# SYNCC-IN/hyperscanning-signal-analysis

Hardware: AMD Instinct MI355X
Metric: MVAR+ffDTF windows/sec, 2x32-ch dyad p=8, 256 freqs (higher is better)
Workload: dtype f64; 1 GPU; C2: 1 dyad(s)/GPU, 2x32 ch @500 Hz, 10 min, 2 s windows 50% overlap (599 windows per dyad), MVAR p=8, 256 freqs 0.5-128 Hz; dyads_per_gpu=1, k1=hop blocks summed once, shared by the overlapping windows (hop 500), k2=block Levinson-Whittle recursion, one workgroup per window, one launch, normalisation=inside K3 (rows of window w by workgroups of window w+lag), parallelism=dyad-sharded x1, gather=none

## Files before the change

### hyperscanning_signal_analysis_amd/csrc/capi.hip

```cpp
#include "../../include/hypermvar.h"
#include "hmv_kernels.h"

#include <atomic>
#include <cmath>
#include <cstdio>
#include <cstdlib>
#include <cstring>

namespace {
thread_local char g_err[256] = "";

int fail(int code, const char* msg) {
  snprintf(g_err, sizeof(g_err), "%s", msg);
  return code;
}
int pad_of(int m) { return (m < 1 || m > HMV_MAX_CHANNELS) ? -1 : ((m + 15) / 16) * 16; }
inline hipStream_t S(void* s) { return reinterpret_cast<hipStream_t>(s); }
inline size_t align256(size_t b) { return (b + 255) & ~size_t(255); }

constexpr int N_TUNE = 6;
struct TuneRange { long long lo, hi; };
constexpr TuneRange kTuneRange[N_TUNE] = {{0, 0}, {0, 1 << 20}, {0, 3}, {0, 2}, {0, 4}, {0, 140000}};
long long env_knob(const char* name, int key) {
  const char* e = getenv(name);
// ... 741 lines not shown
      hmv::LagcovEnsArgs ea{};
      ea.x = a.x; ea.rec_stride = a.rec_stride; ea.ld = a.ld; ea.T = a.ens->T;
      ea.trial_rec = reinterpret_cast<const long long*>(a.ens->trial_rec);
      ea.trial_start = reinterpret_cast<const long long*>(a.ens->trial_start);
      ea.group_ptr = reinterpret_cast<const long long*>(a.ens->group_ptr);
      ea.item_group = reinterpret_cast<const long long*>(a.item_rec + i0);
      ea.item_offset = reinterpret_cast<const long long*>(a.item_start + i0);
      ea.n_items = c; ea.m = a.m; ea.n = a.n; ea.p = a.p; ea.R = R;
      if (ens_shared) {
        ea.it0 = i0; ea.nwin = a.grid_nwin; ea.hop = a.grid_hop; ea.k = (int)(a.n / a.grid_hop); ea.Q = Qb;
      }
      if (a.ens->split) {
        ea.trial_rec_b = reinterpret_cast<const long long*>(a.ens->trial_rec_b);
        ea.trial_start_b = reinterpret_cast<const long long*>(a.ens->trial_start_b);
        ea.split = a.ens->split; ea.R_base = a.ens->R_base;
        ea.item_base = a.ens->item_base ? reinterpret_cast<const long long*>(a.ens->item_base + i0) : nullptr;
        rc = hmv::launch_lagcov_ensemble_split(ea, mp, st0);
      } else {
        rc = hmv::launch_lagcov_ensemble(ea, mp, ens_shared, st0);
      }
    } else if (a.pairs) {
      hmv::LagcovPairsArgs pa{};
      pa.x = a.x; pa.rec_stride = a.rec_stride; pa.ld = a.ld;
      pa.rec_a = reinterpret_cast<const long long*>(a.item_rec + i0);
      pa.rec_b = reinterpret_cast<const long long*>(a.pairs->rec_b + i0);
      pa.item_start = reinterpret_cast<const long long*>(a.item_start + i0);
      pa.n_items = c; pa.m = a.m; pa.n = a.n; pa.p = a.p; pa.split = a.pairs->split; pa.R = R;
      pa.R_base = a.pairs->R_base;
      pa.base_a = a.pairs->R_base ? reinterpret_cast<const long long*>(a.pairs->base_a + i0) : nullptr;
      pa.base_b = a.pairs->R_base ? reinterpret_cast<const long long*>(a.pairs->base_b + i0) : nullptr;
      rc = hmv::launch_lagcov_pairs(pa, mp, st0);
    } else if (a.mix) {
      hmv::LagcovMixArgs ma{};
      ma.Rt = a.mix->Rt; ma.W = a.mix->W; ma.scale = a.mix->scale; ma.n_trials = a.mix->n_trials; ma.n_win = a.mix->n_win;
      ma.it0 = i0; ma.n_items = c; ma.m = a.m; ma.m_pad = mp; ma.p = a.p; ma.R = R;
      rc = hmv::launch_lagcov_mix(ma, st0);
    } else if (regular) {
      for (int64_t it = i0; it < i0 + c && rc == 0;) {
        const int64_t rec = it / a.grid_nwin, w0 = it - rec * a.grid_nwin;
        const int64_t run = ((a.grid_nwin - w0) < (i0 + c - it)) ? (a.grid_nwin - w0) : (i0 + c - it);
        rc = hmv_lagcov_regular_f64(a.x + rec * a.rec_stride, a.ld, a.grid_T, a.grid_first + w0 * a.grid_hop, a.grid_hop,
                                    run, a.m, a.n, a.p, R + (size_t)(it - i0) * (a.p + 1) * t, Qb, st0);
        it += run;
      }
    } else {
      rc = hmv_lagcov_f64(a.x, a.rec_stride, a.ld, a.item_rec + i0, a.item_start + i0, c, a.m, a.n, a.p, R, st0);
    }
    if (rc) break;
    if (automatic) {
      hmv::YwArgs ya{};
      ya.R = R; ya.n_items = c; ya.m = a.m; ya.p = a.p; ya.ws = ws; ya.ar = ar_c; ya.V = V_c; ya.info = a.info_yw + i0;
      ya.tiled = -1;
      hmv::YwAutoArgs sel{};
      sel.n = a.n; sel.crit_c = crit_factor(a.crit, a.n); sel.order_out = a.order_out + i0;
      sel.crit_out = a.crit_out ? a.crit_out + (size_t)i0 * a.p : nullptr;
      rc = hmv::launch_yw_auto(ya, sel, mp, st0);
      if (rc) break;
    }
    const bool ldl = (a.flags & (HMV_FLAG_YW_TILED | HMV_FLAG_YW_ONE_LAUNCH)) || hmv::tuning(HMV_TUNE_YW_FORM) == 1;
    const bool tiled = (a.flags & HMV_FLAG_YW_TILED) || (ldl && !(a.flags & HMV_FLAG_YW_ONE_LAUNCH) && mp == 64 && c >= 128);
    const int64_t yw_flags = (a.flags & ~(int64_t)(HMV_FLAG_YW_TILED | HMV_FLAG_YW_ONE_LAUNCH)) |
                             (ldl ? (tiled ? HMV_FLAG_YW_TILED : HMV_FLAG_YW_ONE_LAUNCH) : 0);
    const int64_t c0 = (split && tiled && c >= 16) ? (c + 1) / 2 : c, c1 = c - c0;
    if (c1 > 0 && !automatic) {
      int hrc = (int)hipEventRecord(fj->fork, st0);
      if (!hrc) hrc = (int)hipStreamWaitEvent(st1, fj->fork, 0);
      if (hrc) { rc = hrc; break; }
      rc = hmv_yw_solve_f64(R + (size_t)c0 * (a.p + 1) * t, c1, a.m, a.p, ws + (size_t)c0 * ws_item,
                            ar_c + (size_t)c0 * t * a.p, V_c + (size_t)c0 * t, nullptr, a.info_yw + i0 + c0, yw_flags, st1);
      hrc = (int)hipEventRecord(fj->join, st1);
      if (!hrc) hrc = (int)hipStreamWaitEvent(st0, fj->join, 0);
      if (hrc) {
        (void)hipStreamSynchronize(st1);
        if (!rc) rc = hrc;
      }
      if (rc) break;
    }
    const int64_t yw_form = hmv::tuning(HMV_TUNE_YW_FORM);
    const bool from_tiles = !automatic && !a.ar_out && !ldl && (yw_form == 0 || yw_form == 2) && a.measure == MEAS_FFDTF;
    if (!automatic && from_tiles) {
      hmv::YwArgs ya{};
      ya.R = R; ya.n_items = c0; ya.m = a.m; ya.p = a.p; ya.ws = ws; ya.ar = ar_c; ya.V = V_c; ya.info = a.info_yw + i0;
      ya.tiled = -1; ya.no_emit = 1;
      rc = hmv::launch_yw(ya, mp, st0);
    } else if (!automatic) {
      rc = hmv_yw_solve_f64(R, c0, a.m, a.p, ws, ar_c, V_c, nullptr, a.info_yw + i0, yw_flags, st0);
    }
    if (rc) break;
    const bool last = (ci == n_chunks - 1);
    double* Hc = a.S_out ? reinterpret_cast<double*>(base + w.off_H) : nullptr;
    double* full_c = (a.measure == MEAS_FFDTF) ? nullptr
                     : bands ? reinterpret_cast<double*>(base + w.off_full) : a.ffdtf + (size_t)i0 * a.m * a.m * a.F;
    if (a.measure == MEAS_GPDC) {
      rc = hmv::launch_gpdc_sliding(ar_c, V_c, tw, full_c, c, a.F, a.m, mp, a.p, st0);
    } else {
      rc = tf_ffdtf_impl(a.who, ar_c, c, a.m, a.p, tw, a.F,
                         k3_bands ? nullptr : (full_c ? full_c : a.ffdtf + (size_t)i0 * a.m * a.m * a.F),
                         k3_bands ? a.band_out + (size_t)i0 * a.m * a.m * a.n_bands : nullptr, a.bin_lo, a.bin_hi,
                         a.n_bands, den, Hc, a.info_tf + (size_t)i0 * a.F, a.pivot_tau, tfws, tfws_bytes, a.flags,
                         last ? a.ev_k3_start : nullptr, last ? a.ev_k3_stop : nullptr, st0, from_tiles ? ws : nullptr);
    }
    if (!rc && a.measure == MEAS_DDTF) {
      hmv::DdtfArgs da{};
      da.ar = ar_c; da.V = V_c; da.info_yw = a.info_yw + i0;
      da.B = reinterpret_cast<double*>(base + w.off_B); da.G = reinterpret_cast<double*>(base + w.off_G);
      da.freqs = a.freqs; da.fs = a.fs; da.ff = full_c; da.out = full_c;
      da.n_items = c; da.F = a.F; da.m = a.m; da.p = a.p;
      rc = hmv::launch_ddtf_sliding(da, mp, st0);
    }
    if (!rc && a.measure != MEAS_FFDTF && bands)
      rc = hmv::launch_band_sums(full_c, reinterpret_cast<const int*>(a.bin_lo), reinterpret_cast<const int*>(a.bin_hi),
                                 a.band_out + (size_t)i0 * a.m * a.m * a.n_bands, c * (long long)a.m * a.m, a.F,
                                 a.n_bands, st0);
    if (!rc && a.S_out) {
      hmv::SpecArgs sa;
      sa.H = Hc; sa.V = V_c; sa.S = nullptr; sa.S_mmf = a.S_out + (size_t)i0 * a.m * a.m * a.F * 2;
      sa.n_items = c; sa.F = a.F; sa.m = a.m; sa.sym = 1;
      rc = hmv::launch_spectra(sa, mp, st0);
    }
  }
  return rc;
}
}

int64_t hmv_sliding_bands_workspace_bytes(int64_t chunk, int m, int p, int F) { return sliding_bytes(chunk, m, p, F, 1); }

int hmv_sliding_ffdtf_f64(const double* x, int64_t rec_stride, int64_t ld, const int64_t* item_rec,
                          const int64_t* item_start, int64_t n_items, int m, int n, int p,
                          const double* freqs, int F, double fs, double* ffdtf, double* ar_out, double* V_out,
                          int32_t* info_yw, int32_t* info_tf, void* workspace, int64_t workspace_bytes,
                          int64_t chunk, double pivot_tau, int64_t flags, int64_t grid_hop, int64_t grid_first,
                          int64_t grid_nwin, int64_t grid_T, void* ev_k3_start, void* ev_k3_stop, void* stream,
                          void* aux_stream) {
  SlidingArgs a{"hmv_sliding_ffdtf_f64"};
  a.x = x; a.rec_stride = rec_stride; a.ld = ld; a.item_rec = item_rec; a.item_start = item_start; a.n_items = n_items;
  a.m = m; a.n = n; a.p = p; a.freqs = freqs; a.F = F; a.fs = fs;
  a.ffdtf = ffdtf;
  a.ar_out = ar_out; a.V_out = V_out; a.info_yw = info_yw; a.info_tf = info_tf;
  a.workspace = workspace; a.workspace_bytes = workspace_bytes; a.chunk = chunk; a.pivot_tau = pivot_tau; a.flags = flags;
  a.grid_hop = grid_hop; a.grid_first = grid_first; a.grid_nwin = grid_nwin; a.grid_T = grid_T;
  a.ev_k3_start = ev_k3_start; a.ev_k3_stop = ev_k3_stop;
  a.stream = stream; a.aux_stream = aux_stream;
  return sliding_impl(a);
}

int hmv_sliding_ffdtf_bands_f64(const double* x, int64_t rec_stride, int64_t ld, const int64_t* item_rec,
                                const int64_t* item_start, int64_t n_items, int m, int n, int p,
                                const double* freqs, int F, double fs, double* band_out, const int32_t* bin_lo,
                                const int32_t* bin_hi, int n_bands, double* ar_out, double* V_out,
                                int32_t* info_yw, int32_t* info_tf, void* workspace, int64_t workspace_bytes,
                                int64_t chunk, double pivot_tau, int64_t flags, int64_t grid_hop, int64_t grid_first,
                                int64_t grid_nwin, int64_t grid_T, void* ev_k3_start, void* ev_k3_stop, void* stream,
                                void* aux_stream) {
  if (!band_out && n_items != 0) return fail(-4, "hmv_sliding_ffdtf_bands_f64: null pointer / empty grid");
  SlidingArgs a{"hmv_sliding_ffdtf_bands_f64"};
  a.x = x; a.rec_stride = rec_stride; a.ld = ld; a.item_rec = item_rec; a.item_start = item_start; a.n_items = n_items;
  a.m = m; a.n = n; a.p = p; a.freqs = freqs; a.F = F; a.fs = fs;
  a.band_out = band_out; a.bin_lo = bin_lo; a.bin_hi = bin_hi; a.n_bands = n_bands;
  a.ar_out = ar_out; a.V_out = V_out; a.info_yw = info_yw; a.info_tf = info_tf;
  a.workspace = workspace; a.workspace_bytes = workspace_bytes; a.chunk = chunk; a.pivot_tau = pivot_tau; a.flags = flags;
  a.grid_hop = grid_hop; a.grid_first = grid_first; a.grid_nwin = grid_nwin; a.grid_T = grid_T;
  a.ev_k3_start = ev_k3_start; a.ev_k3_stop = ev_k3_stop;
  a.stream = stream; a.aux_stream = aux_stream;
  return sliding_impl(a);
}

// ... 486 lines not shown
```

### hyperscanning_signal_analysis_amd/csrc/hmv_kernels.h

```cpp
#pragma once
#include <hip/hip_runtime.h>
#include <stdint.h>

namespace hmv {

long long tuning(int key);

struct LagcovArgs {
  const double* x;
  long long rec_stride;
  long long ld;
  const long long* item_rec;
  const long long* item_start;
  long long n_items;
  int m, n, p;
  double* R;
  int blocks;
  long long blk_first, blk_T;
};
int launch_lagcov(const LagcovArgs& a, int m_pad, hipStream_t st);
struct LagcombArgs {
  const double* Q;
  const double* x;
  long long ld, first, hop, T;
  long long n_win;
  int k, m, p;
  double* R;
};
int launch_lagcomb(const LagcombArgs& a, int m_pad, hipStream_t st);
struct LagcovEnsArgs {
  const double* x;
  long long rec_stride, ld;
  long long T;
  const long long* trial_rec;
  const long long* trial_start;
  const long long* group_ptr;
  const long long* item_group;
  const long long* item_offset;
  long long n_items;
  int m, n, p;
  double* R;
  long long it0, nwin, hop;
  int k;
  double* Q;
  const long long* trial_rec_b;
  const long long* trial_start_b;
  int split;
  const double* R_base;
  const long long* item_base;
};
bool lagcov_ensemble_shared_ok(int n, long long hop, int p, int max_k);
long long lagcov_ensemble_q_tiles(long long n_items, long long nwin, int k);
int launch_lagcov_ensemble(const LagcovEnsArgs& a, int m_pad, bool shared, hipStream_t st);
int launch_lagcov_ensemble_split(const LagcovEnsArgs& a, int m_pad, hipStream_t st);
struct LagcovPairsArgs {
  const double* x;
  long long rec_stride, ld;
  const long long* rec_a;
  const long long* rec_b;
  const long long* item_start;
  long long n_items;
  int m, n, p, split;
  double* R;
  const double* R_base;
  const long long* base_a;
  const long long* base_b;
};
int launch_lagcov_pairs(const LagcovPairsArgs& a, int m_pad, hipStream_t st);
struct LagcovMixArgs {
  const double* Rt;
  const double* W;
  const double* scale;
  long long n_trials, n_win;
  long long it0, n_items;
  int m, m_pad, p;
  double* R;
};
int launch_lagcov_mix(const LagcovMixArgs& a, hipStream_t st);

struct YwArgs {
  const double* R;
  long long n_items;
  int m, p;
  double* ws;
  double* ar;
  double* V;
  double* Vq_logdet;
  int* info;
  int tiled;
  int only_guarded;
  const int* order;
  int no_emit;
};
struct YwAutoArgs {
  int n;
  double crit_c;
  int* order_out;
  double* crit_out;
};
long long yw_ws_tiles(int p);
int launch_yw(const YwArgs& a, int m_pad, hipStream_t st);
int launch_yw_lwr(const YwArgs& a, int m_pad, hipStream_t st);
int launch_yw_lwr2(const YwArgs& a, int m_pad, hipStream_t st);
int launch_yw_auto(const YwArgs& a, const YwAutoArgs& s, int m_pad, hipStream_t st);
int launch_yw_guarded(const YwArgs& a, int m_pad, hipStream_t st);

struct TfArgs {
  const double* ar;
  const double* arx;
  const double* tw;
  const double* Zin;
  double* detph;
  double* P;
  double* rowsum;
  double* H;
  double* A;
  int* info;
  long long n_items;
  int F, p, m;
  double tau;
  double* ff;
  double* den;
  int* wcount;
  int* ready;
  int* missed;
  long long fuse_items;
  int lag;
  double* bands;
  const int* band_lo;
  const int* band_hi;
  int nb;
  unsigned long long* stamps;
};
int launch_twiddles(const double* freqs, int F, double fs, int p, double* tw, hipStream_t st);
int launch_tf_inv(const TfArgs& a, int m_pad, hipStream_t st, hipEvent_t ev_start = nullptr, hipEvent_t ev_stop = nullptr,
                  const double* yw_ws = nullptr);
int launch_cinv(const TfArgs& a, int m_pad, hipStream_t st);
long long tf_workspace_doubles(long long n_items, int m_pad, int p);
int tf_band_max_F(int m_pad);

struct NormArgs {
  const double* P;
  const double* rowsum;
  double* den;
  double* out;
  long long n_items;
  int F, m, m_pad;
  int normalise;
};
int launch_ffdtf_norm(const NormArgs& a, hipStream_t st);

int launch_trial_mean(const double* in, double* out, long long n, int trials, hipStream_t st);
int launch_ddtf(const double* ff, const double* kappa, double* out, long long n, hipStream_t st);
int launch_band_sums(const double* in, const int* lo, const int* hi, double* out, long long rows, int F, int nb,
                     hipStream_t st);

int launch_transpose_c128(const double* in, double* out, long long n_items, int F, int m, int m_pad, hipStream_t st);

struct SpecArgs {
  const double* H;
  const double* V;
  double* S;
  double* S_mmf;
  long long n_items;
  int F, m;
  int sym;
};
int launch_spectra(const SpecArgs& a, int m_pad, hipStream_t st);

int launch_pack_c128(const double* in, double* out, long long n_items, int F, int m, int m_pad, hipStream_t st);
int launch_pcoh(const double* Sinv, const double* detph, double* out, long long n_items, int F, int m, int m_pad, hipStream_t st);
int launch_gpdc(const double* A, const double* V, double* out, long long n_items, int F, int m, int m_pad, hipStream_t st);

struct DdtfArgs {
  const double* ar;
// ... 101 lines not shown
```

### hyperscanning_signal_analysis_amd/csrc/tf_inv.hip

```cpp
#include "hmv_common.h"
#include "hmv_kernels.h"

namespace hmv {

#ifndef HMV_K3_WGS
#define HMV_K3_WGS 4
#endif

#ifndef HMV_ROW_LOADS_SC1
#define HMV_ROW_LOADS_SC1 0
#endif

#define HMV_LDS_FENCE()                                     \
  do {                                                      \
    __builtin_amdgcn_fence(__ATOMIC_RELEASE, "wavefront");  \
    __builtin_amdgcn_wave_barrier();                        \
    __builtin_amdgcn_fence(__ATOMIC_ACQUIRE, "wavefront");  \
  } while (0)

#ifdef HMV_STAMP
#define HMV_T(idx)                                                                     \
  do {                                                                                 \
    __builtin_amdgcn_sched_barrier(0);                                                 \
    unsigned long long t_;                                                             \
// ... 788 lines not shown
                      , tsum, tlast
#endif
  );
}

#ifndef HMV_K3A_INC
#define HMV_K3A_INC "tf_inv64_body.inc"
#endif
#include HMV_K3A_INC
#ifndef HMV_K3A_WGS
#ifdef HMV_STAMP
#define HMV_K3A_WGS 4
#else
#define HMV_K3A_WGS 5
#endif
#endif
static_assert(K3A_PBUF == 0 && K3A_NBUF == 16 * TfLds<4>::PBUF && K3A_RSUM == 16 * (TfLds<4>::TOTAL - TfLds<4>::RSUM),
              "LDS map of the generated body and of the epilogue disagree");

__global__ void __launch_bounds__(256, HMV_K3A_WGS) tf_inv64_asm_kernel(TfArgs a) {
  constexpr int NT = 4;
  __shared__ __attribute__((aligned(16))) unsigned char lds[K3A_LDS_TOTAL];
  int* s_orig = reinterpret_cast<int*>(lds + K3A_SORIG);
  int* s_flag = reinterpret_cast<int*>(lds + K3A_SINFO);
  const int wv = uni(threadIdx.x >> 6);
  const int w = (wv + (int)((blockIdx.x * 2654435761u) >> 20)) % NT;
  const int item = uni((int)(blockIdx.x / (unsigned)a.F));
  const int f = uni((int)(blockIdx.x - (unsigned)item * (unsigned)a.F));
  const long long gw = (long long)item * a.F + f;
  if (w == 0) {
    const int l = lane_id();
    s_orig[l] = l;
    if (l == 0) *s_flag = 0;
  }
  const int p = a.p, P2 = (p + 1) >> 1;
  const double* arx = a.arx + ((size_t)item * NT + w) * (size_t)(16 * 64 * 2) * P2;
  const double* tw = a.tw + (size_t)f * p * 2;
  const double tau = a.tau;
  const unsigned ldsbase = (unsigned)(uintptr_t)lds;
  double acc[32];
#ifdef HMV_STAMP
  unsigned long long tsum[8] = {0, 0, 0, 0, 0, 0, 0, 0}, tlast = 0, q0, q1, q2, q3;
  unsigned tl32;
  K3A_BODY_STAMPED(acc, arx, tw, p, w, tau, ldsbase, q0, q1, q2, q3, tl32);
  {
    const unsigned long long d[8] = {q0 & 0xffffffffull, q0 >> 32, q1 & 0xffffffffull, q1 >> 32,
                                     q2 & 0xffffffffull, q2 >> 32, q3 & 0xffffffffull, q3 >> 32};
    tsum[0] = d[0]; tsum[2] = d[1]; tsum[3] = d[2] + d[3] + d[4]; tsum[1] = d[5] + d[6] + d[7];
    unsigned long long now;
    asm volatile("s_memtime %0\n\ts_waitcnt lgkmcnt(0)" : "=s"(now)::"memory");
    tlast = (now & ~0xffffffffull) | tl32;
    if (tlast > now) tlast -= 0x100000000ull;
    if (a.stamps && lane_id() == 0) {
      unsigned long long* det = a.stamps + ((size_t)a.n_items * a.F * NT + (size_t)(gw * NT + wv)) * 8;
      for (int k = 0; k < 8; ++k) det[k] = d[k];
    }
  }
#else
  K3A_BODY(acc, arx, tw, p, w, tau, ldsbase);
#endif
  double re[NT][4], im[NT][4];
#pragma unroll
  for (int Ig = 0; Ig < 4; ++Ig)
#pragma unroll
    for (int Jl = 0; Jl < 4; ++Jl) {
      re[Ig][Jl] = acc[2 * (4 * Ig + Jl)];
      im[Ig][Jl] = acc[2 * (4 * Ig + Jl) + 1];
    }
  double2* smem = reinterpret_cast<double2*>(lds);
  double* rsum = reinterpret_cast<double*>(lds + K3A_RSUM);
  tf_outputs<NT, false>(a, item, f, gw, w, wv, re, im, smem, rsum, s_orig, s_flag, nullptr
#ifdef HMV_STAMP
                        , tsum, tlast
#endif
  );
}

template <int NT, bool TILES>
__global__ void __launch_bounds__(256) ar_pack_kernel(const double* ar, const double* ws, long long ws_item, double* arx,
                                                      long long n_items, int p) {
  constexpr int MP = 16 * NT;
  const int P2 = (p + 1) >> 1;
  const long long per_item = (long long)MP * MP * P2;
  const long long idx = (long long)blockIdx.x * 256 + threadIdx.x;
  if (idx >= n_items * per_item) return;
  const long long item = idx / per_item;
  long long r = idx - item * per_item;
  const int lane = (int)(r & 63); r >>= 6;
  const int h = (int)(r % P2); r /= P2;
  const int Jl = (int)(r & 3); r >>= 2;
  const int Ig = (int)(r % NT);
  const int w = (int)(r / NT);
  const int row = 16 * Ig + 4 * ((lane >> 2) & 3) + (lane >> 4), col = 4 * (Jl * NT + w) + (lane & 3);
  double2 v;
  if (TILES && reinterpret_cast<const int*>(ws + (size_t)(item + 1) * ws_item)[-1] == 0) {
    const double* e = ws + (size_t)item * ws_item + ((size_t)(p & 1) * p + 2 * h) * (MP * MP) + (size_t)row * MP + col;
    v.x = e[0];
    v.y = (2 * h + 1 < p) ? e[MP * MP] : 0.0;
  } else {
    const double* e = ar + ((size_t)item * MP * MP + (size_t)row * MP + col) * p;
    v.x = e[2 * h];
    v.y = (2 * h + 1 < p) ? e[2 * h + 1] : 0.0;
  }
  reinterpret_cast<double2*>(arx)[idx] = v;
}

__global__ void twiddle_kernel(const double* freqs, int F, double fs, int p, double* tw) {
  const int idx = blockIdx.x * blockDim.x + threadIdx.x;
  if (idx >= F * p) return;
  const int f = idx / p, k = idx - f * p;
  const double c = (double)(-(k + 1) * 2) * 3.141592653589793;
  const double th = c * freqs[f] / fs;
  double s, co;
  sincos(th, &s, &co);
  tw[2 * idx] = co;
  tw[2 * idx + 1] = s;
}

int launch_twiddles(const double* freqs, int F, double fs, int p, double* tw, hipStream_t st) {
  const int n = F * p;
  hipLaunchKernelGGL(twiddle_kernel, dim3((n + 255) / 256), dim3(256), 0, st, freqs, F, fs, p, tw);
  return (int)hipGetLastError();
}

int tf_band_max_F(int m_pad) {
  switch (m_pad) {
    case 16: return (2 * TfLds<1>::TOTAL) & ~31;
    case 32: return (2 * TfLds<2>::TOTAL) & ~31;
    case 48: return (2 * TfLds<3>::TOTAL) & ~31;
    case 64: return (2 * TfLds<4>::TOTAL) & ~31;
  }
  return 0;
}

long long tf_workspace_doubles(long long n_items, int m_pad, int p) {
  return n_items * (long long)m_pad * m_pad * 2 * ((p + 1) / 2);
}

int launch_tf_inv(const TfArgs& a_in, int m_pad, hipStream_t st, hipEvent_t ev_start, hipEvent_t ev_stop,
                  const double* yw_ws) {
  TfArgs a = a_in;
  if (a.n_items == 0 || a.F == 0) return 0;
  const bool fused = ((a.ff != nullptr || a.bands != nullptr) && a.fuse_items > 0);
  if (fused) {
    if (!a.P || !a.den || !a.wcount || !a.ready || !a.missed || a.lag < 1) return -3;
    if (a.bands && (!a.band_lo || !a.band_hi || a.nb < 1 || a.F % 32 != 0 || a.F > tf_band_max_F(m_pad) || a.A)) return -3;
    if (const hipError_t e = hipMemsetAsync(a.wcount, 0, sizeof(int) * (2 * (size_t)a.n_items + 1), st)) return (int)e;
  } else {
    a.ff = nullptr;
    a.bands = nullptr;
  }
  const long long n = a.n_items * (long long)a.F;
  const dim3 grid((unsigned)n);
  const long long slots = a.n_items * (long long)m_pad * m_pad * ((a.p + 1) / 2);
  const dim3 pgrid((unsigned)((slots + 255) / 256));
  double* arx = const_cast<double*>(a.arx);
  const long long ws_item = yw_ws_tiles(a.p) * (long long)m_pad * m_pad;
#define HMV_AR_PACK(NT)                                                                                                  \
  if (yw_ws) hipLaunchKernelGGL((ar_pack_kernel<NT, true>), pgrid, dim3(256), 0, st, a.ar, yw_ws, ws_item, arx, a.n_items, a.p); \
  else hipLaunchKernelGGL((ar_pack_kernel<NT, false>), pgrid, dim3(256), 0, st, a.ar, yw_ws, ws_item, arx, a.n_items, a.p)
  switch (m_pad) {
    case 16: HMV_AR_PACK(1); break;
    case 32: HMV_AR_PACK(2); break;
    case 48: HMV_AR_PACK(3); break;
    case 64: HMV_AR_PACK(4); break;
    default: return -1;
  }
#undef HMV_AR_PACK
  if (ev_start)
    if (const hipError_t e = hipEventRecord(ev_start, st)) return (int)e;
  switch (m_pad) {
    case 16: hipLaunchKernelGGL((tf_inv_kernel<1, false>), grid, dim3(64), 0, st, a); break;
    case 32: hipLaunchKernelGGL((tf_inv_kernel<2, false>), grid, dim3(128), 0, st, a); break;
    case 48: hipLaunchKernelGGL((tf_inv_kernel<3, false>), grid, dim3(192), 0, st, a); break;
    case 64:
      if (tuning(5) > 0) {
        (void)hipFuncSetAttribute(reinterpret_cast<const void*>(&tf_inv64_asm_kernel), hipFuncAttributeMaxDynamicSharedMemorySize,
                                  (int)tuning(5));
        (void)hipFuncSetAttribute(reinterpret_cast<const void*>(&tf_inv_kernel<4, false>),
                                  hipFuncAttributeMaxDynamicSharedMemorySize, (int)tuning(5));
      }
      if ((tuning(3 ) != 1 || a.bands != nullptr) && a.A == nullptr)
        hipLaunchKernelGGL(tf_inv64_asm_kernel, grid, dim3(256), (unsigned)tuning(5 ), st, a);
      else
        hipLaunchKernelGGL((tf_inv_kernel<4, false>), grid, dim3(256), (unsigned)tuning(5), st, a);
      break;
  }
  if (ev_stop)
    if (const hipError_t e = hipEventRecord(ev_stop, st)) return (int)e;
  if (fused) {
    const long long tail_rows = (a.fuse_items > a.lag ? a.lag : a.fuse_items) * a.m;
    const dim3 mgrid((unsigned)(tail_rows > 2048 ? 2048 : (tail_rows < 256 ? 256 : tail_rows)));
    switch (m_pad) {
      case 16: hipLaunchKernelGGL(norm_missed_kernel<1>, mgrid, dim3(64), 0, st, a); break;
      case 32: hipLaunchKernelGGL(norm_missed_kernel<2>, mgrid, dim3(128), 0, st, a); break;
      case 48: hipLaunchKernelGGL(norm_missed_kernel<3>, mgrid, dim3(192), 0, st, a); break;
      case 64: hipLaunchKernelGGL(norm_missed_kernel<4>, mgrid, dim3(256), 0, st, a); break;
    }
  }
  return (int)hipGetLastError();
}

int launch_cinv(const TfArgs& a_in, int m_pad, hipStream_t st) {
  TfArgs a = a_in;
  a.ff = nullptr;
  a.bands = nullptr;
  a.fuse_items = 0;
  const long long n = a.n_items * (long long)a.F;
  if (n == 0) return 0;
  const dim3 grid((unsigned)n);
  switch (m_pad) {
    case 16: hipLaunchKernelGGL((tf_inv_kernel<1, true>), grid, dim3(64), 0, st, a); break;
    case 32: hipLaunchKernelGGL((tf_inv_kernel<2, true>), grid, dim3(128), 0, st, a); break;
    case 48: hipLaunchKernelGGL((tf_inv_kernel<3, true>), grid, dim3(192), 0, st, a); break;
    case 64: hipLaunchKernelGGL((tf_inv_kernel<4, true>), grid, dim3(256), 0, st, a); break;
    default: return -1;
  }
  return (int)hipGetLastError();
}

}
```

### hyperscanning_signal_analysis_amd/csrc/yw_lwr_core.h

```cpp
#pragma once
#include "yw_common.h"

namespace hmv {

#ifndef HMV_LWR_GUARD
#define HMV_LWR_GUARD 1e-7
#endif

template <int NT, bool VQ, bool AUTO, bool LEGACY = false>
__device__ __forceinline__ void yw_lwr_body(const YwArgs& a, const YwAutoArgs& sel) {
  static_assert(VQ || !AUTO, "the selecting form needs every log det Vf_q");
  constexpr int MP = 16 * NT, KH = MP / 2, SH = KH + 6, NIW = NT, NJ = NT, TILE = MP * MP;
  constexpr int NV = (MP * KH / 2 + 255) / 256;
  constexpr int SI = YwCfg<NT>::S;
  constexpr bool ONE0 = !LEGACY && !AUTO;
  constexpr int GEMM_D = 2 * MP * SH, INV_D = MP * SI, BUF_D = GEMM_D > INV_D ? GEMM_D : INV_D;
  __shared__ __attribute__((aligned(16))) double buf[BUF_D];
  __shared__ double Pb[2 * MP * 4];
  __shared__ double Nb[4 * MP * 4];
  __shared__ int s_info;
  __shared__ double s_ld[4];
  __shared__ double s_pm[4 + 4 * 4];
  __shared__ int s_guard;
  __shared__ double s_logdet, s_best;
// ... 61 lines not shown
        if (NV * 256 == MP * KH / 2 || idx < MP * KH / 2) {
          const unsigned off = !tr ? ((idx / PR) * MP + 2 * (idx % PR)) * 8u : ((idx / PT) * MP + 2 * (idx % PT)) * 8u;
          const unsigned cb = !tr ? kh * KH * 8u : kh * KH * MP * 8u;
          v[r] = *reinterpret_cast<const f64x2 __attribute__((address_space(1)))*>(gptr(src, cb, off));
        }
      }
    }
  };
  auto park = [&](double* dst, const f64x2 (&v)[NV], bool tr) __attribute__((always_inline)) {
    const unsigned t = tid();
#pragma unroll
    for (int r = 0; r < NV; ++r) {
      const unsigned idx = RSTEP ? t : t + 256 * r;
      if (NV * 256 == MP * KH / 2 || t + 256 * r < MP * KH / 2) {
        if (!tr) {
          double* d = dst + (RSTEP ? r * (256 / PR) * SH : 0) + ((idx / PR) * SH + 2 * (idx % PR));
          d[0] = v[r].x;
          d[1] = v[r].y;
        } else {
          double* d = dst + (RSTEP ? r * (256 / PT) : 0) + ((2 * (idx % PT)) * SH + idx / PT);
          d[0] = v[r].x;
          d[SH] = v[r].y;
        }
      }
    }
  };
  auto park_strip = [&](const double (&v)[NIW][NJ], int kh) __attribute__((always_inline)) {
    const unsigned l = lane(), i = l >> 4, cc = l & 15;
    double* d = Xh + (unsigned)(4 * wv * NT) * SH + (i * SH + cc);
#pragma unroll
    for (int ii = 0; ii < NIW; ++ii)
#pragma unroll
      for (int J = 0; J < NJ; ++J) {
        const int c0 = 16 * J - kh * KH;
        if (c0 >= 0 && c0 + 15 < KH) d[4 * ii * SH + c0] = v[ii][J];
        else if (c0 + 15 >= 0 && c0 < KH) {
          const int col = c0 + (int)cc;
          if (col >= 0 && col < KH) d[4 * ii * SH + c0] = v[ii][J];
        }
      }
  };
#ifndef HMV_LWR_GEMM_PIPE
#define HMV_LWR_GEMM_PIPE 1
#endif
  auto gemm_half = [&](double (&acc)[NIW][NJ]) __attribute__((always_inline)) {
    const unsigned l = lane();
    const double* xa = Xh + (unsigned)(4 * wv * NT) * SH + ((l & 3) * SH + (l >> 4));
    const double* yb = Yh + ((l & 15) * SH + (l >> 4));
#if HMV_LWR_GEMM_PIPE
    constexpr int NS = KH / 4;
    double av[2][NIW], bv[2][NJ];
    auto rd = [&](int set, int k0) __attribute__((always_inline)) {
#pragma unroll
      for (int ii = 0; ii < NIW; ++ii) av[set][ii] = xa[4 * ii * SH + k0];
#pragma unroll
      for (int J = 0; J < NJ; ++J) bv[set][J] = yb[16 * J * SH + k0];
    };
    rd(0, 0);
    static_for<NS>([&](auto sc) __attribute__((always_inline)) {
      constexpr int s = decltype(sc)::value, cur = s & 1;
      if constexpr (s + 1 < NS) rd(cur ^ 1, 4 * (s + 1));
      __builtin_amdgcn_sched_barrier(0);
#pragma unroll
      for (int ii = 0; ii < NIW; ++ii)
#pragma unroll
        for (int J = 0; J < NJ; ++J) acc[ii][J] = mfma4(av[cur][ii], bv[cur][J], acc[ii][J]);
      __builtin_amdgcn_sched_barrier(0);
    });
#else
#pragma unroll 2
    for (int k0 = 0; k0 < KH; k0 += 4) {
      double av[NIW], bv[NJ];
#pragma unroll
      for (int ii = 0; ii < NIW; ++ii) av[ii] = xa[4 * ii * SH + k0];
#pragma unroll
      for (int J = 0; J < NJ; ++J) bv[J] = yb[16 * J * SH + k0];
#pragma unroll
      for (int ii = 0; ii < NIW; ++ii)
#pragma unroll
        for (int J = 0; J < NJ; ++J) acc[ii][J] = mfma4(av[ii], bv[J], acc[ii][J]);
    }
#endif
  };
  auto product = [&](double (&acc)[NIW][NJ], const double* srcX, bool trX, const double (&xr)[NIW][NJ], const double* srcY,
                     bool trY) __attribute__((always_inline)) {
    f64x2 vx[NV], vy[NV];
    if (srcX) fetch(vx, srcX, 0, trX);
    fetch(vy, srcY, 0, trY);
    __syncthreads();
    if (srcX) park(Xh, vx, trX); else park_strip(xr, 0);
    park(Yh, vy, trY);
    if (srcX) fetch(vx, srcX, 1, trX);
    fetch(vy, srcY, 1, trY);
    __syncthreads();
    gemm_half(acc);
    __syncthreads();
    if (srcX) park(Xh, vx, trX); else park_strip(xr, 1);
    park(Yh, vy, trY);
    __syncthreads();
    gemm_half(acc);
  };
  auto store_tile = [&](double* dst, const double (&v)[NIW][NJ]) __attribute__((always_inline)) {
    const unsigned l = lane(), off = ((l >> 4) * MP + (l & 15)) * 8u;
    const double* strip = dst + (unsigned)(4 * wv * NT) * MP;
#pragma unroll
    for (int ii = 0; ii < NIW; ++ii)
#pragma unroll
      for (int J = 0; J < NJ; ++J)
        *(double __attribute__((address_space(1)))*)(gptr(strip, (4 * ii * MP + 16 * J) * 8u, off)) = v[ii][J];
  };
  auto load_tile = [&](double (&v)[NIW][NJ], const double* src, bool tr) __attribute__((always_inline)) {
    const unsigned l = lane(), off = !tr ? ((l >> 4) * MP + (l & 15)) * 8u : ((l & 15) * MP + (l >> 4)) * 8u;
    const double* strip = src + (unsigned)(4 * wv * NT) * (!tr ? MP : 1);
#pragma unroll
    for (int ii = 0; ii < NIW; ++ii)
#pragma unroll
      for (int J = 0; J < NJ; ++J) {
        const unsigned cb = !tr ? (4 * ii * MP + 16 * J) * 8u : (16 * J * MP + 4 * ii) * 8u;
        v[ii][J] = *reinterpret_cast<const double __attribute__((address_space(1)))*>(gptr(strip, cb, off));
      }
  };
  auto sub = [&](double (&g)[NIW][NJ], const double (&acc)[NIW][NJ]) __attribute__((always_inline)) {
#pragma unroll
    for (int ii = 0; ii < NIW; ++ii)
#pragma unroll
      for (int J = 0; J < NJ; ++J) g[ii][J] -= acc[ii][J];
  };
  auto invert = [&](const double (&g)[NIW][NJ], double* out, double* logdet, int q) __attribute__((always_inline)) {
    const int info_base = q * MP;
    const int l = lane(), i = l >> 4, cc = l & 15;
    __syncthreads();
#pragma unroll
    for (int ii = 0; ii < NIW; ++ii)
#pragma unroll
      for (int J = 0; J < NJ; ++J) buf[(4 * (wv * NT + ii) + i) * SI + 16 * J + cc] = g[ii][J];
    __syncthreads();
    spd_inverse_coop<NT, SI>(buf, Pb, Nb, &s_info, s_ld, out, logdet, info_base, s_pm, a.m);
    if (threadIdx.x == 0 && !(s_pm[0] >= HMV_LWR_GUARD * s_pm[1])) {
      if (!AUTO) s_guard = 1;
      else if (s_guard == 0) s_guard = q + 1;
    }
    __syncthreads();
  };

  auto invert2 = [&](const double (&ga)[NIW][NJ], const double (&gb)[NIW][NJ], double* out_a, double* out_b, double* logdet_b,
                     int q) __attribute__((always_inline)) {
    const int info_base = q * MP;
    spd_inverse_coop2<NT, SI>(ga, gb, buf, Pb, Nb, &s_info, s_ld, out_a, out_b, logdet_b, info_base, s_pm, a.m);
    if (threadIdx.x == 0 && (!(s_pm[0] >= HMV_LWR_GUARD * s_pm[1]) || !(s_pm[2] >= HMV_LWR_GUARD * s_pm[3]))) {
      if (!AUTO) s_guard = 1;
      else if (s_guard == 0) s_guard = q + 1;
    }
    __syncthreads();
  };

  auto ld_dst = [&](int q) __attribute__((always_inline)) -> double* {
    if (AUTO) return &s_logdet;
    return a.Vq_logdet + (size_t)item * p + (q - 1);
  };
  auto emit = [&](const double* Aq, int q) __attribute__((always_inline)) {
    double* ar = a.ar + (size_t)item * TILE * p;
    const int total = TILE * q, de = 256 / q, dk = 256 - de * q;
    int e = (int)threadIdx.x / q, k = (int)threadIdx.x - e * q;
    for (int idx = threadIdx.x; idx < total; idx += 256) {
      ar[(size_t)e * p + k] = Aq[(size_t)k * TILE + e];
      e += de;
      k += dk;
      if (k >= q) {
        k -= q;
        ++e;
      }
    }
  };
  auto select = [&](int q) __attribute__((always_inline)) {
    if (threadIdx.x == 0) {
      const double ld = s_logdet;
      const double crit = ld + ((sel.crit_c * (double)q) * (double)(a.m * a.m)) / (double)sel.n;
      if (sel.crit_out) sel.crit_out[(size_t)item * p + (q - 1)] = crit;
      if (a.Vq_logdet) a.Vq_logdet[(size_t)item * p + (q - 1)] = ld;
      const int take = (crit < s_best) ? 1 : 0;
      if (take) {
        s_best = crit;
        s_qstar = q;
      }
      s_take = take;
    }
    __syncthreads();
    if (s_take) {
      emit(Agen[q & 1], q);
      double* Vo = a.V + (size_t)item * TILE;
      for (int idx = threadIdx.x; idx < TILE; idx += 256) Vo[idx] = Vf[idx];
    }
  };

  double g[NIW][NJ], acc[NIW][NJ], dacc[NIW][NJ];
  const double (&none)[NIW][NJ] = g;
  if (!ONE0) {
    load_tile(g, R, false);
    store_tile(Vf, g);
    store_tile(Vb, g);
    load_tile(g, R + TILE, true);
    store_tile(Dq, g);
  } else {
    load_tile(g, R + TILE, true);
    store_tile(Dq, g);
  }
  __syncthreads();
  for (int q = 0; q < p; ++q) {
    const double* Ao = Agen[q & 1];
    const double* Bo = Bgen[q & 1];
    double* An = Agen[(q + 1) & 1];
    double* Bn = Bgen[(q + 1) & 1];
    const bool last = (q == p - 1);
    const bool one0 = ONE0 && q == 0;
    load_tile(g, one0 ? R : Vb, false);
#ifndef HMV_LWR_SINGLE_INVERSES
    if (!one0 && (!last || (VQ && q >= 1))) {
      load_tile(acc, Vf, false);
      invert2(g, acc, VbI, VfI, (VQ && q >= 1) ? ld_dst(q) : nullptr, q);
    } else {
      invert(g, VbI, nullptr, q);
    }
#else
    invert(g, VbI, nullptr, q);
    if (!one0 && (!last || (VQ && q >= 1))) {
      load_tile(g, Vf, false);
      invert(g, VfI, (VQ && q >= 1) ? ld_dst(q) : nullptr, q);
    }
#endif
    if (AUTO && q >= 1) select(q);
    zero(acc);
    product(acc, Dq, false, none, VbI, false);
    store_tile(An + (size_t)q * TILE, acc);
    zero(dacc);
    product(dacc, nullptr, false, acc, Dq, false);
    load_tile(g, one0 ? R : Vf, false);
    sub(g, dacc);
    store_tile(Vf, g);
    if (!last) {
      zero(acc);
      product(acc, Dq, true, none, one0 ? VbI : VfI, false);
      store_tile(Bn + (size_t)q * TILE, acc);
      zero(dacc);
      product(dacc, nullptr, false, acc, Dq, true);
      load_tile(g, one0 ? R : Vb, false);
      sub(g, dacc);
      store_tile(Vb, g);
    }
    __syncthreads();
    zero(dacc);
    for (int k = 0; k < q; ++k) {
      const int j = LEGACY ? k : q - 1 - k;
      zero(acc);
      product(acc, An + (size_t)q * TILE, false, none, Bo + (size_t)(q - 1 - k) * TILE, true);
      load_tile(g, Ao + (size_t)k * TILE, false);
      sub(g, acc);
      store_tile(An + (size_t)k * TILE, g);
      if (!last) {
        product(dacc, nullptr, false, g, R + (size_t)(q + 1 - k) * TILE, false);
        zero(acc);
        product(acc, Bn + (size_t)q * TILE, false, none, Ao + (size_t)(q - 1 - j) * TILE, true);
        load_tile(g, Bo + (size_t)j * TILE, false);
        sub(g, acc);
        store_tile(Bn + (size_t)j * TILE, g);
      }
    }
    if (!last) {
      product(dacc, An + (size_t)q * TILE, false, none, R + TILE, false);
      load_tile(g, R + (size_t)(q + 2) * TILE, true);
      sub(g, dacc);
      store_tile(Dq, g);
    }
    __syncthreads();
  }
  if (VQ) {
    load_tile(g, Vf, false);
    invert(g, VfI, ld_dst(p), p);
  }
  if (AUTO) {
    select(p);
    __syncthreads();
    const int bad = s_info, qs = bad ? 0 : s_qstar;
    if (threadIdx.x == 0) {
      a.info[item] = bad ? bad : (qs == 0 ? -1 : 0);
      sel.order_out[item] = qs;
      *yw_guard_ptr(a.ws, item, p, TILE) = (bad == 0 && qs > 0 && s_guard != 0 && s_guard - 1 <= qs) ? 1 : 0;
    }
    double* ar = a.ar + (size_t)item * TILE * p;
    const int total = TILE * p, dk = 256 % p;
    int k = (int)threadIdx.x % p;
    for (int idx = threadIdx.x; idx < total; idx += 256) {
      if (k >= qs) ar[idx] = 0.0;
      k += dk;
      k = (k >= p) ? k - p : k;
    }
    if (qs == 0) {
      double* Vo = a.V + (size_t)item * TILE;
      for (int idx = threadIdx.x; idx < TILE; idx += 256) Vo[idx] = R[idx];
    }
    return;
  }
  load_tile(g, Vf, false);
  store_tile(a.V + (size_t)item * TILE, g);
  if (threadIdx.x == 0) {
    a.info[item] = s_info;
    *yw_guard_ptr(a.ws, item, p, TILE) = (s_info == 0) ? s_guard : 0;
  }
  if (LEGACY || !a.no_emit) emit(Agen[p & 1], p);
}

}
```

Measured before the change: 60860 windows/s.

## Skip unused final Vf update, pipeline LWR product fetches, tile ar_pack via LDS

Adds a no_V flag so the block Levinson-Whittle kernel skips the last-order forward noise covariance update and its store when neither V nor S is requested. It restructures the product helper so the next product's first global fetch can be issued before the current second gemm half, behind a compile-time HMV_LWR_PRODUCT_PIPE switch that defaults off. The ar_pack kernel in the tiles path now runs one workgroup per 16-row tile, staging rows through shared memory with double2 loads before scattering into the packed layout, which replaces per-element strided gathers. The pipelining adds register pressure if enabled, and the skipped V means V_c is left unwritten when unused.

```diff
diff --git a/hyperscanning_signal_analysis_amd/csrc/capi.hip b/hyperscanning_signal_analysis_amd/csrc/capi.hip
--- a/hyperscanning_signal_analysis_amd/csrc/capi.hip
+++ b/hyperscanning_signal_analysis_amd/csrc/capi.hip
@@ -847,6 +847,7 @@
       hmv::YwArgs ya{};
       ya.R = R; ya.n_items = c0; ya.m = a.m; ya.p = a.p; ya.ws = ws; ya.ar = ar_c; ya.V = V_c; ya.info = a.info_yw + i0;
       ya.tiled = -1; ya.no_emit = 1;
+      ya.no_V = (!a.V_out && !a.S_out) ? 1 : 0;
       rc = hmv::launch_yw(ya, mp, st0);
     } else if (!automatic) {
       rc = hmv_yw_solve_f64(R, c0, a.m, a.p, ws, ar_c, V_c, nullptr, a.info_yw + i0, yw_flags, st0);
diff --git a/hyperscanning_signal_analysis_amd/csrc/hmv_kernels.h b/hyperscanning_signal_analysis_amd/csrc/hmv_kernels.h
--- a/hyperscanning_signal_analysis_amd/csrc/hmv_kernels.h
+++ b/hyperscanning_signal_analysis_amd/csrc/hmv_kernels.h
@@ -91,6 +91,7 @@
   int only_guarded;
   const int* order;
   int no_emit;
+  int no_V;
 };
 struct YwAutoArgs {
   int n;
diff --git a/hyperscanning_signal_analysis_amd/csrc/tf_inv.hip b/hyperscanning_signal_analysis_amd/csrc/tf_inv.hip
--- a/hyperscanning_signal_analysis_amd/csrc/tf_inv.hip
+++ b/hyperscanning_signal_analysis_amd/csrc/tf_inv.hip
@@ -894,27 +894,52 @@
   constexpr int MP = 16 * NT;
   const int P2 = (p + 1) >> 1;
   const long long per_item = (long long)MP * MP * P2;
-  const long long idx = (long long)blockIdx.x * 256 + threadIdx.x;
-  if (idx >= n_items * per_item) return;
-  const long long item = idx / per_item;
-  long long r = idx - item * per_item;
-  const int lane = (int)(r & 63); r >>= 6;
-  const int h = (int)(r % P2); r /= P2;
-  const int Jl = (int)(r & 3); r >>= 2;
-  const int Ig = (int)(r % NT);
-  const int w = (int)(r / NT);
-  const int row = 16 * Ig + 4 * ((lane >> 2) & 3) + (lane >> 4), col = 4 * (Jl * NT + w) + (lane & 3);
-  double2 v;
-  if (TILES && reinterpret_cast<const int*>(ws + (size_t)(item + 1) * ws_item)[-1] == 0) {
-    const double* e = ws + (size_t)item * ws_item + ((size_t)(p & 1) * p + 2 * h) * (MP * MP) + (size_t)row * MP + col;
-    v.x = e[0];
-    v.y = (2 * h + 1 < p) ? e[MP * MP] : 0.0;
+  if constexpr (TILES) {
+    constexpr int SR = MP + 2;
+    __shared__ __attribute__((aligned(16))) double t[2][16][SR];
+    const int Ig = (int)(blockIdx.x % NT), h = (int)((blockIdx.x / NT) % P2);
+    const long long item = blockIdx.x / (NT * P2);
+    if (item >= n_items) return;
+    const bool two = 2 * h + 1 < p;
+    if (reinterpret_cast<const int*>(ws + (size_t)(item + 1) * ws_item)[-1] == 0) {
+      const double* src = ws + (size_t)item * ws_item + ((size_t)(p & 1) * p + 2 * h) * (MP * MP) + (size_t)16 * Ig * MP;
+      for (int idx = threadIdx.x; idx < 16 * MP / 2; idx += 256) {
+        const int row = idx / (MP / 2), c = 2 * (idx % (MP / 2));
+        *reinterpret_cast<double2*>(&t[0][row][c]) = reinterpret_cast<const double2*>(src)[idx];
+        *reinterpret_cast<double2*>(&t[1][row][c]) = two ? reinterpret_cast<const double2*>(src + MP * MP)[idx] : double2{0.0, 0.0};
+      }
+    } else {
+      const double* src = ar + ((size_t)item * MP * MP + (size_t)16 * Ig * MP) * p;
+      for (int idx = threadIdx.x; idx < 16 * MP; idx += 256) {
+        const double* e = src + (size_t)idx * p;
+        t[0][idx / MP][idx % MP] = e[2 * h];
+        t[1][idx / MP][idx % MP] = two ? e[2 * h + 1] : 0.0;
+      }
+    }
+    __syncthreads();
+    for (int s = threadIdx.x; s < 4 * NT * 64; s += 256) {
+      const int lane = s & 63, Jl = (s >> 6) & 3, w = s >> 8;
+      const int row = 4 * ((lane >> 2) & 3) + (lane >> 4), col = 4 * (Jl * NT + w) + (lane & 3);
+      const long long slot = item * per_item + ((((long long)(w * NT + Ig) * 4 + Jl) * P2 + h) * 64 + lane);
+      reinterpret_cast<double2*>(arx)[slot] = double2{t[0][row][col], t[1][row][col]};
+    }
   } else {
+    const long long idx = (long long)blockIdx.x * 256 + threadIdx.x;
+    if (idx >= n_items * per_item) return;
+    const long long item = idx / per_item;
+    long long r = idx - item * per_item;
+    const int lane = (int)(r & 63); r >>= 6;
+    const int h = (int)(r % P2); r /= P2;
+    const int Jl = (int)(r & 3); r >>= 2;
+    const int Ig = (int)(r % NT);
+    const int w = (int)(r / NT);
+    const int row = 16 * Ig + 4 * ((lane >> 2) & 3) + (lane >> 4), col = 4 * (Jl * NT + w) + (lane & 3);
     const double* e = ar + ((size_t)item * MP * MP + (size_t)row * MP + col) * p;
+    double2 v;
     v.x = e[2 * h];
     v.y = (2 * h + 1 < p) ? e[2 * h + 1] : 0.0;
-  }
-  reinterpret_cast<double2*>(arx)[idx] = v;
+    reinterpret_cast<double2*>(arx)[idx] = v;
+  }
 }
 
 __global__ void twiddle_kernel(const double* freqs, int F, double fs, int p, double* tw) {
@@ -968,8 +993,9 @@
   const dim3 pgrid((unsigned)((slots + 255) / 256));
   double* arx = const_cast<double*>(a.arx);
   const long long ws_item = yw_ws_tiles(a.p) * (long long)m_pad * m_pad;
+  const dim3 tgrid((unsigned)(a.n_items * ((a.p + 1) / 2) * (m_pad / 16)));
 #define HMV_AR_PACK(NT)                                                                                                  \
-  if (yw_ws) hipLaunchKernelGGL((ar_pack_kernel<NT, true>), pgrid, dim3(256), 0, st, a.ar, yw_ws, ws_item, arx, a.n_items, a.p); \
+  if (yw_ws) hipLaunchKernelGGL((ar_pack_kernel<NT, true>), tgrid, dim3(256), 0, st, a.ar, yw_ws, ws_item, arx, a.n_items, a.p); \
   else hipLaunchKernelGGL((ar_pack_kernel<NT, false>), pgrid, dim3(256), 0, st, a.ar, yw_ws, ws_item, arx, a.n_items, a.p)
   switch (m_pad) {
     case 16: HMV_AR_PACK(1); break;
diff --git a/hyperscanning_signal_analysis_amd/csrc/yw_lwr_core.h b/hyperscanning_signal_analysis_amd/csrc/yw_lwr_core.h
--- a/hyperscanning_signal_analysis_amd/csrc/yw_lwr_core.h
+++ b/hyperscanning_signal_analysis_amd/csrc/yw_lwr_core.h
@@ -167,22 +167,37 @@
     }
 #endif
   };
+#ifndef HMV_LWR_PRODUCT_PIPE
+#define HMV_LWR_PRODUCT_PIPE 0
+#endif
+  constexpr bool PIPE = HMV_LWR_PRODUCT_PIPE && !LEGACY;
+  f64x2 vx[NV], vy[NV];
+  auto head = [&](bool xreg, const double* srcX, bool trX, const double* srcY, bool trY) __attribute__((always_inline)) {
+    if (!xreg) fetch(vx, srcX, 0, trX);
+    fetch(vy, srcY, 0, trY);
+  };
+  auto no_next = [&]() __attribute__((always_inline)) {};
   auto product = [&](double (&acc)[NIW][NJ], const double* srcX, bool trX, const double (&xr)[NIW][NJ], const double* srcY,
-                     bool trY) __attribute__((always_inline)) {
-    f64x2 vx[NV], vy[NV];
-    if (srcX) fetch(vx, srcX, 0, trX);
-    fetch(vy, srcY, 0, trY);
-    __syncthreads();
-    if (srcX) park(Xh, vx, trX); else park_strip(xr, 0);
-    park(Yh, vy, trY);
-    if (srcX) fetch(vx, srcX, 1, trX);
-    fetch(vy, srcY, 1, trY);
+                     bool trY, bool xreg, bool pre, auto&& next) __attribute__((always_inline)) {
+    f64x2 lx[NV], ly[NV];
+    f64x2 (&ux)[NV] = PIPE ? vx : lx;
+    f64x2 (&uy)[NV] = PIPE ? vy : ly;
+    if (!PIPE || !pre) {
+      if (!xreg) fetch(ux, srcX, 0, trX);
+      fetch(uy, srcY, 0, trY);
+    }
+    __syncthreads();
+    if (!xreg) park(Xh, ux, trX); else park_strip(xr, 0);
+    park(Yh, uy, trY);
+    if (!xreg) fetch(ux, srcX, 1, trX);
+    fetch(uy, srcY, 1, trY);
     __syncthreads();
     gemm_half(acc);
     __syncthreads();
-    if (srcX) park(Xh, vx, trX); else park_strip(xr, 1);
-    park(Yh, vy, trY);
-    __syncthreads();
+    if (!xreg) park(Xh, ux, trX); else park_strip(xr, 1);
+    park(Yh, uy, trY);
+    __syncthreads();
+    if (PIPE) next();
     gemm_half(acc);
   };
   auto store_tile = [&](double* dst, const double (&v)[NIW][NJ]) __attribute__((always_inline)) {
@@ -280,6 +295,7 @@
 
   double g[NIW][NJ], acc[NIW][NJ], dacc[NIW][NJ];
   const double (&none)[NIW][NJ] = g;
+  const bool NOV = !LEGACY && !VQ && !AUTO && a.no_V != 0;
   if (!ONE0) {
     load_tile(g, R, false);
     store_tile(Vf, g);
@@ -314,20 +330,37 @@
     }
 #endif
     if (AUTO && q >= 1) select(q);
+    const bool skipV = NOV && last;
+    double* Anq = An + (size_t)q * TILE;
+    double* Bnq = Bn + (size_t)q * TILE;
+    auto head_lower0 = [&]() __attribute__((always_inline)) {
+      if (q > 0) head(false, Anq, false, Bo + (size_t)(q - 1) * TILE, true);
+    };
     zero(acc);
-    product(acc, Dq, false, none, VbI, false);
-    store_tile(An + (size_t)q * TILE, acc);
-    zero(dacc);
-    product(dacc, nullptr, false, acc, Dq, false);
-    load_tile(g, one0 ? R : Vf, false);
-    sub(g, dacc);
-    store_tile(Vf, g);
+    product(acc, Dq, false, none, VbI, false, false, false, [&]() __attribute__((always_inline)) {
+      if (!skipV) head(true, nullptr, false, Dq, false);
+    });
+    store_tile(Anq, acc);
+    if (!skipV) {
+      zero(dacc);
+      product(dacc, nullptr, false, acc, Dq, false, true, true, [&]() __attribute__((always_inline)) {
+        if (!last) head(false, Dq, true, one0 ? VbI : VfI, false);
+        else head_lower0();
+      });
+      load_tile(g, one0 ? R : Vf, false);
+      sub(g, dacc);
+      store_tile(Vf, g);
+    }
     if (!last) {
       zero(acc);
-      product(acc, Dq, true, none, one0 ? VbI : VfI, false);
-      store_tile(Bn + (size_t)q * TILE, acc);
+      product(acc, Dq, true, none, one0 ? VbI : VfI, false, false, true,
+              [&]() __attribute__((always_inline)) { head(true, nullptr, false, Dq, true); });
+      store_tile(Bnq, acc);
       zero(dacc);
-      product(dacc, nullptr, false, acc, Dq, true);
+      product(dacc, nullptr, false, acc, Dq, true, true, true, [&]() __attribute__((always_inline)) {
+        if (q > 0) head_lower0();
+        else head(false, Anq, false, R + TILE, false);
+      });
       load_tile(g, one0 ? R : Vb, false);
       sub(g, dacc);
       store_tile(Vb, g);
@@ -336,22 +369,31 @@
     zero(dacc);
     for (int k = 0; k < q; ++k) {
       const int j = LEGACY ? k : q - 1 - k;
+      auto head_after = [&]() __attribute__((always_inline)) {
+        if (last) { if (k + 1 < q) head(false, Anq, false, Bo + (size_t)(q - 2 - k) * TILE, true); }
+        else if (k + 1 == q) head(false, Anq, false, R + TILE, false);
+      };
       zero(acc);
-      product(acc, An + (size_t)q * TILE, false, none, Bo + (size_t)(q - 1 - k) * TILE, true);
+      product(acc, Anq, false, none, Bo + (size_t)(q - 1 - k) * TILE, true, false, k > 0 ? last : !skipV,
+              [&]() __attribute__((always_inline)) {
+                if (!last) head(true, nullptr, false, R + (size_t)(q + 1 - k) * TILE, false);
+                else head_after();
+              });
       load_tile(g, Ao + (size_t)k * TILE, false);
       sub(g, acc);
       store_tile(An + (size_t)k * TILE, g);
       if (!last) {
-        product(dacc, nullptr, false, g, R + (size_t)(q + 1 - k) * TILE, false);
+        product(dacc, nullptr, false, g, R + (size_t)(q + 1 - k) * TILE, false, true, true,
+                [&]() __attribute__((always_inline)) { head(false, Bnq, false, Ao + (size_t)(q - 1 - j) * TILE, true); });
         zero(acc);
-        product(acc, Bn + (size_t)q * TILE, false, none, Ao + (size_t)(q - 1 - j) * TILE, true);
+        product(acc, Bnq, false, none, Ao + (size_t)(q - 1 - j) * TILE, true, false, true, head_after);
         load_tile(g, Bo + (size_t)j * TILE, false);
         sub(g, acc);
         store_tile(Bn + (size_t)j * TILE, g);
       }
     }
     if (!last) {
-      product(dacc, An + (size_t)q * TILE, false, none, R + TILE, false);
+      product(dacc, Anq, false, none, R + TILE, false, false, true, no_next);
       load_tile(g, R + (size_t)(q + 2) * TILE, true);
       sub(g, dacc);
       store_tile(Dq, g);
@@ -385,8 +427,10 @@
     }
     return;
   }
-  load_tile(g, Vf, false);
-  store_tile(a.V + (size_t)item * TILE, g);
+  if (!NOV) {
+    load_tile(g, Vf, false);
+    store_tile(a.V + (size_t)item * TILE, g);
+  }
   if (threadIdx.x == 0) {
     a.info[item] = s_info;
     *yw_guard_ptr(a.ws, item, p, TILE) = (s_info == 0) ? s_guard : 0;
```

Result: no change. 60870 windows/s (median of 2 runs) (+0.0%).
